# CristianSimion5/vk-raytracing-engine

Hardware: AMD Instinct MI355X
Metric: Mrays/s (higher is better)
Workload: dtype f32

## Files before the change

### include/vkrt.h

```cpp
#ifndef VKRT_H
#define VKRT_H

#include <stdint.h>
#include "vkrt_host_device.h"

#ifdef __cplusplus
extern "C" {
#endif

#define VKRT_ABI_VERSION 4

enum vkrt_status {
  VKRT_OK = 0,
  VKRT_ERR_INVALID_ARGUMENT = 1,
  VKRT_ERR_NO_DEVICE = 2,
  VKRT_ERR_HIP = 3,
  VKRT_ERR_OUT_OF_MEMORY = 4,
  VKRT_ERR_NOT_BUILT = 5,
  VKRT_ERR_UNSUPPORTED = 6
};

typedef struct vkrt_scene vkrt_scene;

typedef struct vkrt_prim_mesh {
// ... 67 lines not shown
typedef struct vkrt_counters {
  uint64_t rays_closest;
  uint64_t rays_shadow;
  uint64_t hits;
  uint64_t diffuse_hits;
  uint64_t tex_taps;
  uint64_t pixels;
  uint64_t nodes_visited;
  uint64_t tris_tested;
  uint64_t wave_node_steps;
  uint64_t wave_tri_steps;
  uint64_t traversal_faults;
  uint64_t pair_records;
} vkrt_counters;

typedef struct vkrt_accel_info {
  uint32_t triangle_count;
  uint32_t node_count;
  uint32_t max_depth;
  uint32_t build_flags;
  float    sah_cost;
  float    build_ms;
  uint64_t node_bytes;
  uint64_t triangle_bytes;
  uint32_t reference_count;
  uint32_t reserved;
} vkrt_accel_info;

int         vkrt_abi_version(void);
const char* vkrt_last_error(void);
int         vkrt_device_count(void);

int  vkrt_scene_create(const vkrt_scene_desc* desc, int device, vkrt_scene** out);
void vkrt_scene_destroy(vkrt_scene* scene);

enum vkrt_option {
  VKRT_OPT_MODE            = 1,
  VKRT_OPT_BVH_LAYOUT      = 2,
  VKRT_OPT_WF_SUBFRAMES    = 3,
  VKRT_OPT_WF_TRAV_BLOCK   = 4,
  VKRT_OPT_WF_SHARE        = 5,
  VKRT_OPT_TRI_THRESHOLD   = 6,
  VKRT_OPT_WF_SHARE_PERIOD = 7,
  VKRT_OPT_WF_SHARE_FLAGS  = 8,
  VKRT_OPT_GBUFFER_MIPS    = 9,
  VKRT_OPT_WATERTIGHT      = 10,
  VKRT_OPT_SKIP_DEAD_SHADOW_RAYS = 11,
  VKRT_OPT_ANYHIT_DISSOLVE = 12,
  VKRT_OPT_WF_FRAMES_IN_FLIGHT = 13,
  VKRT_OPT_SPLIT_BUDGET    = 14,
  VKRT_OPT_LAST            = 14,
  VKRT_OPT_WF_SAMPLE_SYNC  = 15,
  VKRT_OPT_WF_CAMERA_ROUNDS = 16,
  VKRT_INFO_ANYHIT_ORDER   = 100,
  VKRT_INFO_SPLIT_BUDGET   = 101
};
int vkrt_scene_set_option(vkrt_scene* scene, int option, int value);
int vkrt_scene_get_option(const vkrt_scene* scene, int option, int* value);

int vkrt_accel_build(vkrt_scene* scene, uint32_t build_flags, void* hip_stream);
int vkrt_accel_get_info(const vkrt_scene* scene, vkrt_accel_info* out);

int vkrt_scene_update_nodes(vkrt_scene* scene, uint32_t first, uint32_t count, const vkrt_node* nodes, void* hip_stream);
int vkrt_accel_refit(vkrt_scene* scene, void* hip_stream);

enum vkrt_memory { VKRT_MEMORY_HOST = 0, VKRT_MEMORY_DEVICE = 1 };
typedef struct vkrt_vertex_update {
  uint32_t struct_size;
  uint32_t first, count;
  uint32_t memory;
  const float* positions;
  const float* normals;
  const float* tangents;
  const float* texcoords0;
} vkrt_vertex_update;
int vkrt_scene_update_vertices(vkrt_scene* scene, const vkrt_vertex_update* update, void* hip_stream);

typedef struct vkrt_ray {
  float origin[3];    float tmin;
  float direction[3]; float tmax;
} vkrt_ray;
typedef struct vkrt_hit {
  float   t, u, v;
  int32_t instance;
  int32_t primitive;
  int32_t prim_mesh;
  int32_t triangle;
  int32_t material;
} vkrt_hit;
int vkrt_intersect(vkrt_scene* scene, const vkrt_ray* rays, uint32_t n, uint32_t anyhit_seed, vkrt_hit* hits, void* hip_stream);
int vkrt_occluded(vkrt_scene* scene, const vkrt_ray* rays, uint32_t n, uint32_t anyhit_seed, int32_t* occluded, void* hip_stream);

enum vkrt_instance_flags {
  VKRT_INSTANCE_FACING_CULL_DISABLE = 0x1,
  VKRT_INSTANCE_FLIP_FACING = 0x2
};
typedef struct vkrt_instance_visibility {
  uint8_t  mask;
  uint8_t  flags;
  uint16_t reserved;
} vkrt_instance_visibility;
int vkrt_scene_set_instance_visibility(vkrt_scene* scene, uint32_t first, uint32_t count, const vkrt_instance_visibility* vis, void* hip_stream);
int vkrt_scene_get_instance_visibility(const vkrt_scene* scene, uint32_t first, uint32_t count, vkrt_instance_visibility* out);

enum vkrt_ray_flags {
  VKRT_RAY_OPAQUE = 0x1,
// ... 134 lines not shown
```

### vk-raytracing-engine_amd/abi.py

```python
import ctypes as C

c_f = C.c_float
c_i = C.c_int32
c_u = C.c_uint32
c_u64 = C.c_uint64


class Mat4(C.Structure):
    _fields_ = [("m", c_f * 16)]


class GlobalUniforms(C.Structure):
    _fields_ = [("viewProj", Mat4), ("viewInverse", Mat4), ("projInverse", Mat4)]


class PushConstantRay(C.Structure):
    _fields_ = [
        ("clearColor", c_f * 4),
        ("frame", c_i),
        ("lightsCount", c_i),
        ("samples", c_i),
        ("depth", c_i),
        ("useShadows", c_i),
        ("useAO", c_i),
# ... 156 lines not shown
class InstanceVisibility(C.Structure):
    _fields_ = [("mask", C.c_uint8), ("flags", C.c_uint8), ("reserved", C.c_uint16)]


class MaterialAlpha(C.Structure):
    _fields_ = [("mode", c_u), ("cutoff", c_f)]


class QueryOpts(C.Structure):
    _fields_ = [("struct_size", c_u), ("ray_flags", c_u), ("cull_mask", c_u), ("anyhit_seed", c_u)]


class PointQuery(C.Structure):
    _fields_ = [("point", c_f * 3), ("radius", c_f)]


class VertexUpdate(C.Structure):
    _fields_ = [("struct_size", c_u), ("first", c_u), ("count", c_u), ("memory", c_u), ("positions", C.c_void_p), ("normals", C.c_void_p),
                ("tangents", C.c_void_p), ("texcoords0", C.c_void_p)]


assert C.sizeof(VertexUpdate) == 48
assert C.sizeof(Ray) == 32
assert C.sizeof(Hit) == 32
assert C.sizeof(Surface) == 128
assert C.sizeof(InstanceVisibility) == 4
assert C.sizeof(QueryOpts) == 16
assert C.sizeof(MaterialAlpha) == 8

assert C.sizeof(GlobalUniforms) == 192
assert C.sizeof(PushConstantRay) == 44
assert C.sizeof(PrimMeshInfo) == 12
assert C.sizeof(GltfPBRMaterial) == 52
assert C.sizeof(GltfLight) == 32
assert C.sizeof(PrimMesh) == 20
assert C.sizeof(Node) == 68

VKRT_OK, VKRT_ERR_INVALID_ARGUMENT, VKRT_ERR_NO_DEVICE, VKRT_ERR_HIP, VKRT_ERR_OUT_OF_MEMORY, VKRT_ERR_NOT_BUILT, VKRT_ERR_UNSUPPORTED = range(7)
VKRT_BUILD_LBVH_GPU = 0x1
VKRT_BUILD_SAH_HOST = 0x2
VKRT_BUILD_PLOC_GPU = 0x4
VKRT_TRACE_SEED_INDEX_ROW_MAJOR = 0x1
VKRT_TRACE_COUNT_TRAVERSAL = 0x2
VKRT_TRACE_TIME_KERNELS = 0x4
VKRT_TRACE_SAME_SEED_EVERY_FRAME = 0x8
VKRT_ABI_VERSION = 4
VKRT_OPT_MODE, VKRT_OPT_BVH_LAYOUT, VKRT_OPT_WF_SUBFRAMES, VKRT_OPT_WF_TRAV_BLOCK = 1, 2, 3, 4
VKRT_OPT_WF_SHARE, VKRT_OPT_TRI_THRESHOLD, VKRT_OPT_WF_SHARE_PERIOD, VKRT_OPT_WF_SHARE_FLAGS = 5, 6, 7, 8
VKRT_OPT_GBUFFER_MIPS = 9
VKRT_OPT_WATERTIGHT, VKRT_OPT_SKIP_DEAD_SHADOW_RAYS, VKRT_OPT_ANYHIT_DISSOLVE = 10, 11, 12
VKRT_OPT_WF_FRAMES_IN_FLIGHT, VKRT_OPT_SPLIT_BUDGET = 13, 14
VKRT_OPT_WF_SAMPLE_SYNC = 15
VKRT_OPT_WF_CAMERA_ROUNDS = 16
VKRT_INFO_ANYHIT_ORDER = 100
VKRT_INFO_SPLIT_BUDGET = 101
VKRT_INSTANCE_FACING_CULL_DISABLE, VKRT_INSTANCE_FLIP_FACING = 0x1, 0x2
VKRT_RAY_OPAQUE, VKRT_RAY_CULL_BACK_FACING, VKRT_RAY_CULL_FRONT_FACING = 0x1, 0x10, 0x20
VKRT_MEMORY_HOST, VKRT_MEMORY_DEVICE = 0, 1
VKRT_SURFACE_GEOMETRY, VKRT_SURFACE_MATERIAL = 0x1, 0x2
VKRT_ALPHA_OPAQUE, VKRT_ALPHA_MASK = 0, 1
VKRT_MULTIHIT_MAX = 16

VKRT_SYMBOLS = [
    "vkrt_abi_version",
    "vkrt_last_error",
    "vkrt_device_count",
    "vkrt_scene_create",
    "vkrt_scene_destroy",
    "vkrt_scene_set_option",
    "vkrt_scene_get_option",
    "vkrt_reserve",
    "vkrt_reserve_frames",
    "vkrt_accel_build",
    "vkrt_accel_get_info",
    "vkrt_scene_update_nodes",
    "vkrt_accel_refit",
    "vkrt_scene_update_vertices",
    "vkrt_intersect",
    "vkrt_occluded",
    "vkrt_scene_set_instance_visibility",
    "vkrt_scene_get_instance_visibility",
    "vkrt_intersect_ex",
    "vkrt_occluded_ex",
    "vkrt_intersect_multi",
    "vkrt_closest_point",
    "vkrt_hit_surface",
    "vkrt_scene_set_material_alpha",
    "vkrt_scene_get_material_alpha",
    "vkrt_shard_rows",
    "vkrt_pathtrace",
    "vkrt_pathtrace_frames",
    "vkrt_gbuffer_raycast",
    "vkrt_hybrid_trace",
    "vkrt_gbuffer_raycast_nrd",
    "vkrt_hybrid_trace_nrd",
    "vkrt_post",
    "vkrt_denoiser_create",
    "vkrt_denoiser_destroy",
    "vkrt_denoiser_reset",
    "vkrt_denoise_diffuse",
    "vkrt_counters_reset",
    "vkrt_counters_read",
    "vkrt_last_trace_ms",
    "vkrt_last_trace_timing",
    "vkrt_debug_check_accel",
    "vkrt_debug_read_accel",
# ... 109 lines not shown
```

### vk-raytracing-engine_amd/csrc/device_scene.h

```cpp
#pragma once
#include <hip/hip_runtime.h>
#include <stddef.h>
#include <stdint.h>
#include "../../include/vkrt_host_device.h"
#include "device_math.h"

struct DevInstance
{
  float o2w[12];
  float w2o[9];
  int32_t primMesh;
  uint32_t vis;
  int32_t pad;
};
static_assert(sizeof(DevInstance) == 96, "DevInstance");
#define VKRT_VIS_CULL_DISABLE 0x100u
#define VKRT_VIS_FLIP 0x200u
#define VKRT_VIS_MIRRORED 0x10000u

#define VKRT_VERTEX_QUADS 3
#define VKRT_VERTEX_BYTES 48u
struct DevTexRef
{
  uint32_t offset;
  uint32_t wh;
  uint32_t flags;
  uint32_t quads;
};
#define VKRT_TEXREF_BASE 0
#define VKRT_TEXREF_MR 1
#define VKRT_TEXREF_NORMAL 2
#define VKRT_TEXREF_EMISSIVE 3
struct DevMaterial
{
  GltfPBRMaterial m;
  int32_t pad;
  uint32_t alphaMode;
  float alphaCutoff;
  DevTexRef tex[4];
};
static_assert(sizeof(DevMaterial) == 128 && offsetof(DevMaterial, alphaMode) == 56, "DevMaterial");
struct DevShadeMaterial
{
  float f[8];
  uint32_t ref[8];
};
static_assert(sizeof(DevShadeMaterial) == 64, "DevShadeMaterial");

#define VKRT_MAX_MIPS 16
struct DevTexture
{
  uint32_t offset;
  uint32_t width, height;
  uint32_t srgb;
};

#define VKRT_NODE_QUADS 4
#define VKRT_LEAF_MAX 8
#define VKRT_TRAV_DONE ((int)0x80000000)

#define VKRT_TRI_QUADS 3

struct DevScene
{
  const float* positions;
  const uint32_t* indices;
  const float4* vertexPN;
  const DevMaterial* materials;
  const DevShadeMaterial* shadeMaterials;
  const GltfLight* lights;
  const DevInstance* instances;
  const DevTexture* textures;
  const uint32_t* texMips;
  const uint32_t* texels;
  const uint4* texQuads;
  const float* srgbLut;
  const float4* nodes;
  const float4* tris;
  const uint4* triShade;
  uint32_t textureCount;
  uint32_t triCount;
  int32_t rootRef;
  uint32_t stackCap;
  uint32_t layout;
  uint32_t stepLimit;
  uint32_t triThreshold;
  uint32_t sharePeriodMask;
  uint32_t shareMinIdle;
  uint32_t gbufferMips;
  uint32_t shareFlags;
  uint32_t watertight;
  float sceneLo[3], sceneHi[3];
  uint32_t dissolve;
  unsigned long long* faults;
};
struct DevQueryScene : DevScene
{
  const uint2* nodeMasks;
  uint32_t cullMask;
  uint32_t rayFlags;
};
struct DevSurfaceScene : DevScene
{
  const uint4* primMeshes;
  uint32_t instanceCount;
};

#define VKRT_TRAV_FAULT(sc) atomicAdd((sc).faults, 1ull)

#ifndef VKRT_W8_MAX_POSTPONED
#define VKRT_W8_MAX_POSTPONED 8
#endif
// ... 44 lines not shown
```

### vk-raytracing-engine_amd/csrc/traverse_share.h

```cpp
#pragma once
#include "traverse_wide.h"

#define VKRT_SHARE_LDS_WORDS 384
struct ShareRes
{
  unsigned long long* key;
  int* slot;
  float* u;
  float* v;
  int* donor;
};
VKRT_DEV void shareSync()
{
  __builtin_amdgcn_fence(__ATOMIC_RELEASE, "wavefront");
  __builtin_amdgcn_wave_barrier();
  __builtin_amdgcn_fence(__ATOMIC_ACQUIRE, "wavefront");
}
VKRT_DEV ShareRes shareRes(int* lds320)
{
  ShareRes r;
  r.key = (unsigned long long*)lds320; r.slot = lds320 + 128; r.u = (float*)(lds320 + 192); r.v = (float*)(lds320 + 256); r.donor = lds320 + 320;
  return r;
}

template <bool COUNT, bool ANYHIT, int TM = 0>
VKRT_DEV void traverse_wide8_share(const DevScene& sc, bool valid, f3 o, f3 d, float tmin, float tmax, uint2* stk, ShareRes res, RayHit& hit,
                                   TravCount& tc, uint32_t raySeed = 0u)
{
  TriRay<(TM & VKRT_TM_WATERTIGHT) != 0> tr;
  tr.set(d);
  const float4* __restrict__ nodes = sc.nodes;
  const float4* __restrict__ tris = sc.tris;
  const int stride = 64;
  const int cap = (int)(sc.stackCap >> 1);
  const int lane = (int)lane_id();
  const unsigned shareMin = sc.shareMinIdle;
  const unsigned long long below = (1ull << lane) - 1ull;
  bool farFirst = ANYHIT && anyhit_far_first(sc, o, d, tmax);

  res.key[lane] = ((unsigned long long)__float_as_uint(tmax) << 32) | 0xffffffffull;
  res.slot[lane] = -1; res.u[lane] = 0.0f; res.v[lane] = 0.0f;
  shareSync();

  int owner = lane;
  f3 id = mk3(safe_inv(d.x), safe_inv(d.y), safe_inv(d.z));
  bool px = !(id.x < 0.0f), py = !(id.y < 0.0f), pz = !(id.z < 0.0f);
  unsigned oct4 = ((px ? 1u : 0u) | (py ? 2u : 0u) | (pz ? 4u : 0u)) * 0x01010101u;
  uint2 G = make_uint2(0u, (valid && sc.rootRef != VKRT_TRAV_DONE) ? 0x80000000u : 0u);
  uint2 T = make_uint2(0u, 0u);
  int sp = 0, sb = 0, nPost = 0;
  unsigned steps = sc.stepLimit;
  bool busy = G.y != 0u;

  for(unsigned iter = 0;; iter++)
  {
    const unsigned long long busyMask = __ballot(busy);
    if(busyMask == 0ull)
      break;
    if((iter & sc.sharePeriodMask) == sc.sharePeriodMask && (unsigned)__popcll(~busyMask) >= shareMin)
    {
      const bool giveStack = busy && sp - sb >= 1;
      const bool giveChild = (sc.shareFlags & 1u) != 0u && busy && !giveStack && (G.y & 0xff000000u & ((G.y & 0xff000000u) - 1u)) != 0u;
      const bool mayTris = (sc.shareFlags & 16u) != 0u && busy && !giveStack && !giveChild;
      const bool giveParked = mayTris && nPost > 0;
      const bool giveTris = mayTris && !giveParked && (T.y & (T.y - 1u)) != 0u;
      const bool wants = giveStack || giveChild || giveParked || giveTris;
      const unsigned long long donorMask = __ballot(wants), idleMask = ~busyMask;
      if(donorMask != 0ull)
      {
        const unsigned n = min((unsigned)__popcll(donorMask), (unsigned)__popcll(idleMask));
        const unsigned giveRank = (unsigned)__popcll(donorMask & below), takeRank = (unsigned)__popcll(idleMask & below);
        const bool gives = wants && giveRank < n;
        const bool takes = !busy && takeRank < n;
        uint2 e = make_uint2(0u, 0u);
        if(gives)
        {
          if(giveStack)
          {
            e = stk[sb * stride];
            sb++;
          }
          else if(giveChild)
          {
            const unsigned top = G.y & 0xff000000u;
            const unsigned low = farFirst ? (0x80000000u >> (unsigned)__clz((int)top)) : (top & (0u - top));
            e = make_uint2(G.x, low | (G.y & 0xffu));
            G.y &= ~low;
          }
          else if(giveParked)
          {
            e = stk[(cap - nPost) * stride];
            e.x |= 0x80000000u;
            nPost--;
          }
          else
          {
            const unsigned lo = (unsigned)__ffs((int)T.y) - 1u, hi = 31u - (unsigned)__clz((int)T.y);
            const unsigned upper = T.y & ~((1u << ((lo + hi + 1u) >> 1)) - 1u);
            e = make_uint2(T.x | 0x80000000u, upper);
            T.y &= ~upper;
          }
          res.donor[giveRank] = lane;
        }
        shareSync();
        const int src = takes ? res.donor[takeRank] : lane;
        const unsigned ex = (unsigned)__shfl((int)e.x, src), ey = (unsigned)__shfl((int)e.y, src);
        const float ox = __shfl(o.x, src), oy = __shfl(o.y, src), oz = __shfl(o.z, src);
        const float dx = __shfl(d.x, src), dy = __shfl(d.y, src), dz = __shfl(d.z, src);
        const float ix = __shfl(id.x, src), iy = __shfl(id.y, src), iz = __shfl(id.z, src);
        const float tm = __shfl(tmax, src);
        const int ow = __shfl(owner, src);
        if(TM & VKRT_TM_DISSOLVE)
        {
          const uint32_t sd = (uint32_t)__shfl((int)raySeed, src);
          if(takes) raySeed = sd;
        }
        if(takes)
        {
          o = mk3(ox, oy, oz); d = mk3(dx, dy, dz); id = mk3(ix, iy, iz); tmax = tm;
          tr.set(d);
          farFirst = ANYHIT && anyhit_far_first(sc, o, d, tmax);
          px = !(id.x < 0.0f); py = !(id.y < 0.0f); pz = !(id.z < 0.0f);
          oct4 = ((px ? 1u : 0u) | (py ? 2u : 0u) | (pz ? 4u : 0u)) * 0x01010101u;
          if(ex & 0x80000000u)
          {
            G = make_uint2(0u, 0u);
            T = make_uint2(ex & 0x7fffffffu, ey);
          }
          else
          {
            G = make_uint2(ex, ey);
            T = make_uint2(0u, 0u);
          }
          sp = 0; sb = 0; nPost = 0;
          owner = ow;
          steps = sc.stepLimit;
          busy = true;
        }
      }
    }
    shareSync();
    if(busy)
    {
      float bt = tmax;
      int bg = -1;
      bool finished = false;
      bool occluded = false;
      if(ANYHIT)
        finished = __hip_atomic_load(&res.slot[owner], __ATOMIC_RELAXED, __HIP_MEMORY_SCOPE_WAVEFRONT) >= 0;
      else
      {
        const unsigned long long k = __hip_atomic_load(&res.key[owner], __ATOMIC_RELAXED, __HIP_MEMORY_SCOPE_WAVEFRONT);
        bt = __uint_as_float((unsigned)(k >> 32));
        bg = (int)(unsigned)k;
      }
      if(!finished)
      {
        struct Cand
        {
          bool found;
          float t, u, v;
          int slot, gid;
        };
        auto testOne = [&](Cand& cd) {
          const unsigned i = (unsigned)__ffs((int)T.y) - 1u;
          T.y &= T.y - 1u;
          const unsigned s = T.x + i;
          const float4* __restrict__ tp = tris + (size_t)s * VKRT_TRI_QUADS;
          const float4 a = tp[0];
          const float4 b = tp[1];
          const float4 c = tp[2];
          if(COUNT)
          {
            tc.tris++;
            if(lane == __ffsll((long long)__ballot(1)) - 1) tc.waveTriSteps++;
          }
          float t, u, v;
          bool ccw;
          if(tr.hit(o, d, a, b, c, t, u, v, ccw) && t > tmin)
          {
            if(ANYHIT)
            {
              if(t < tmax && !cd.found && !query_rejects<TM>(sc, c, ccw) && !anyhit_ignores<TM>(sc, s, c.y, raySeed, VKRT_HOOK_UV(TM, u, v)))
              {
                cd.found = true; cd.t = t; cd.slot = (int)s;
              }
            }
            else
            {
              const int gid = tri_gid<TM>(c.y);
              const float rt = cd.found ? cd.t : bt;
              const int rg = cd.found ? cd.gid : bg;
              if((t < rt || (t == rt && gid < rg)) && !query_rejects<TM>(sc, c, ccw) && !anyhit_ignores<TM>(sc, s, c.y, raySeed, VKRT_HOOK_UV(TM, u, v)))
              {
                cd.found = true; cd.t = t; cd.u = u; cd.v = v; cd.slot = (int)s; cd.gid = gid;
              }
            }
          }
        };
        auto publish = [&](const Cand& cd) {
          if(!cd.found)
            return;
// ... 30 lines not shown
          {
            if(__builtin_expect(sp + nPost >= cap && nPost > VKRT_W8_POSTPONE_ROOM, 0))
            {
              const uint2 keep = T;
              T = stk[(cap - nPost) * stride];
              nPost--;
              flushT();
              T = keep;
            }
            if(sp + nPost < cap)
            {
              stk[sp * stride] = G;
              sp++;
            }
            else
              VKRT_TRAV_FAULT(sc);
          }
          uint2 Tn;
          w8_test_children<COUNT, (TM & VKRT_TM_FILTER) != 0>(nodes, child, o, id, oct4, px, py, pz, tmin, bt, G, Tn, tc, query_node_masks<TM>(sc),
                                                              query_cull_mask<TM>(sc));
          if(Tn.y != 0u)
          {
            if(T.y != 0u)
            {
              if(__builtin_expect(nPost < VKRT_W8_MAX_POSTPONED && sp + nPost < cap, 1))
              {
                nPost++;
                stk[(cap - nPost) * stride] = T;
              }
              else
              {
                if(!occluded)
                  flushT();
                T.y = 0u;
              }
            }
            T = Tn;
          }
        }
        if((G.y & 0xff000000u) == 0u && sp > sb)
        {
          sp--;
          G = stk[sp * stride];
        }
        if(T.y == 0u && nPost > 0)
        {
          T = stk[(cap - nPost) * stride];
          nPost--;
        }
        bool triStep = true;
        if(sc.triThreshold > 1u)
          triStep = (unsigned)__popcll(__ballot(T.y != 0u)) * 64u >= sc.triThreshold * (unsigned)__popcll(busyMask) ||
                    __ballot((G.y & 0xff000000u) != 0u) == 0ull;
        if(T.y != 0u && triStep && !occluded)
        {
          Cand cd = {false, 0.0f, 0.0f, 0.0f, -1, 0};
          testOne(cd);
          publish(cd);
        }
        if(ANYHIT && occluded)
          finished = true;
        else if((G.y & 0xff000000u) == 0u && T.y == 0u && nPost == 0)
          finished = true;
        else if(--steps == 0u)
        {
          VKRT_TRAV_FAULT(sc);
          finished = true;
        }
      }
      if(finished)
        busy = false;
    }
  }
  shareSync();
  hit.t = __uint_as_float((unsigned)(res.key[lane] >> 32)); hit.u = res.u[lane]; hit.v = res.v[lane]; hit.slot = res.slot[lane];
  if(ANYHIT)
    hit.t = tmax;
}
```

### vk-raytracing-engine_amd/csrc/vkrt_api.cpp

```cpp
#include <hip/hip_runtime.h>

#include <algorithm>
#include <chrono>
#include <cmath>
#include <cstdarg>
#include <cstdio>
#include <cstdlib>
#include <cstring>
#include <initializer_list>
#include <string>
#include <vector>

#include "../../include/vkrt.h"
#include "bvh_host.h"
#include "dev_buffer.h"
#include "device_scene.h"
#include "kernels.h"
#include "wide_node.h"

#define VKRT_TRI_THRESHOLD_DEFAULT 32
#define VKRT_WF_SHARE_DEFAULT 16
#define VKRT_WF_SHARE_FLAGS_DEFAULT 25
#define VKRT_WF_FRAMES_IN_FLIGHT_DEFAULT 3
#define VKRT_SPLIT_BUDGET_DEFAULT -1
#define VKRT_WF_SAMPLE_SYNC_DEFAULT 1
#define VKRT_WF_CAMERA_ROUNDS_DEFAULT 1
#include "lbvh.h"
#include "refit.h"
#include "vertex_update.h"

namespace {

thread_local std::string g_lastError;

int fail(int code, const char* fmt, ...)
{
  char buf[512];
  va_list ap;
  va_start(ap, fmt);
  vsnprintf(buf, sizeof buf, fmt, ap);
  va_end(ap);
  g_lastError = buf;
  return code;
}

#define HIP_TRY(expr)                                                      \
  do                                                                       \
  {                                                                        \
    std::string m_;                                                        \
    if(const int rc_ = vkrt::hip_status((expr), #expr, m_); rc_ != VKRT_OK) \
      return fail(rc_, "%s", m_.c_str());                                  \
  } while(0)

}

struct vkrt_scene
{
  int device = 0;
  int cuCount = 256;
  std::vector<float> positions;
  std::vector<uint32_t> indices;
  std::vector<vkrt_prim_mesh> primMeshes;
  std::vector<vkrt_node> nodes;
  uint32_t lightCount = 0, materialCount = 0;
  std::vector<float> materialAlpha;
  std::vector<void*> allocs;
  DevScene dev{};
  vkrt::TreeBuffers accel;
  bool built = false;
  vkrt_accel_info info{};
  unsigned int* workCounter = nullptr;
  DevCounters* counters = nullptr;
  hipEvent_t evStart = nullptr, evStop = nullptr;
  bool timed = false;
  void* wfMem = nullptr;
  WfBuffers wf{};
  WfAsync wfAsync{};
  std::vector<hipEvent_t> wfEvents;
  WfTiming wfTiming{};
  bool wfTimed = false;
  int splitResolved = 0;
  int wfTimingRounds = 0;
  std::vector<hipEvent_t> wfPool;
  int opt[VKRT_OPT_WF_CAMERA_ROUNDS + 1] = {0, 1, 1, 3, 64, VKRT_WF_SHARE_DEFAULT, VKRT_TRI_THRESHOLD_DEFAULT, 0, VKRT_WF_SHARE_FLAGS_DEFAULT, 1, 0, 0, 0,
                                            VKRT_WF_FRAMES_IN_FLIGHT_DEFAULT, VKRT_SPLIT_BUDGET_DEFAULT, VKRT_WF_SAMPLE_SYNC_DEFAULT, VKRT_WF_CAMERA_ROUNDS_DEFAULT};
  bool hasLargeTriangles = false;
  bool wavefront = true;
  bool stale = false;
  bool refitted = false;
  vkrt::RefitScratch refit;
  bool positionsOnDevice = false;
  vkrt::DevBuf vertexStage;
  size_t vertexStageBytes = 0;
  std::vector<vkrt_instance_visibility> vis;
  uint64_t masksPresent[4] = {0, 0, 0, 0};
  vkrt::DevBuf nodeMasks;
  std::vector<vkrt_material_alpha> alpha;
  uint32_t alphaMasks = 0;
  const uint4* surfacePrimMeshes = nullptr;
};

namespace {

template <typename T>
int upload(vkrt_scene* s, const T* src, size_t count, const T** dst)
{
  void* p = nullptr;
  const size_t bytes = std::max<size_t>(count * sizeof(T), 16);
  HIP_TRY(hipMalloc(&p, bytes));
  s->allocs.push_back(p);
  if(count)
    HIP_TRY(hipMemcpy(p, src, count * sizeof(T), hipMemcpyHostToDevice));
  *dst = (const T*)p;
  return VKRT_OK;
}

int checkTransform(const vkrt_node& n, uint32_t i)
{
  for(int k = 0; k < 16; k++)
    if(!std::isfinite(n.worldMatrix[k]))
      return fail(VKRT_ERR_INVALID_ARGUMENT, "node %u: worldMatrix[%d] is not finite", i, k);
  return VKRT_OK;
}

int validate(const vkrt_scene_desc* d)
{
  if(!d)
    return fail(VKRT_ERR_INVALID_ARGUMENT, "desc is NULL");
  if(d->struct_size != sizeof(vkrt_scene_desc))
    return fail(VKRT_ERR_INVALID_ARGUMENT, "vkrt_scene_desc.struct_size %u != %zu (ABI mismatch)", d->struct_size,
                sizeof(vkrt_scene_desc));
  if(d->vertex_count && (!d->positions || !d->normals || !d->tangents || !d->texcoords0))
    return fail(VKRT_ERR_INVALID_ARGUMENT, "vertex arrays missing");
  if(d->index_count && !d->indices)
    return fail(VKRT_ERR_INVALID_ARGUMENT, "indices missing");
  if(d->material_count == 0 || !d->materials)
    return fail(VKRT_ERR_INVALID_ARGUMENT, "at least one material is required (nvh::GltfScene appends a default one)");
  if(d->light_count == 0 || !d->lights)
// ... 28 lines not shown
    const GltfPBRMaterial& m = d->materials[i];
    const int32_t t[4] = {m.pbrBaseColorTexture, m.metallicRoughnessTexture, m.normalTexture, m.emissiveTexture};
    for(int k = 0; k < 4; k++)
      if(t[k] >= (int32_t)d->texture_count && d->texture_count > 0)
        return fail(VKRT_ERR_INVALID_ARGUMENT, "material %u: texture index %d out of range", i, t[k]);
  }
  for(uint32_t i = 0; i < d->texture_count; i++)
    if(!d->textures[i].rgba8 || d->textures[i].width == 0 || d->textures[i].height == 0)
      return fail(VKRT_ERR_INVALID_ARGUMENT, "texture %u: empty", i);
  return VKRT_OK;
}

float srgbEncode(float c) { return c <= 0.0031308f ? 12.92f * c : 1.055f * powf(c, 1.0f / 2.4f) - 0.055f; }
void downsampleLevel(const uint32_t* src, uint32_t sw, uint32_t sh, uint32_t* dst, uint32_t dw, uint32_t dh, bool srgb, const float* lut512)
{
  for(uint32_t y = 0; y < dh; y++)
    for(uint32_t x = 0; x < dw; x++)
    {
      const float fu = ((float)x + 0.5f) * ((float)sw / (float)dw) - 0.5f, fv = ((float)y + 0.5f) * ((float)sh / (float)dh) - 0.5f;
      const float flx = floorf(fu), fly = floorf(fv), ax = fu - flx, ay = fv - fly;
      auto cl = [](int v, int n) { return v < 0 ? 0 : (v >= n ? n - 1 : v); };
      const int x0 = cl((int)flx, (int)sw), x1 = cl((int)flx + 1, (int)sw), y0 = cl((int)fly, (int)sh), y1 = cl((int)fly + 1, (int)sh);
      const uint32_t p[4] = {src[(size_t)y0 * sw + x0], src[(size_t)y0 * sw + x1], src[(size_t)y1 * sw + x0], src[(size_t)y1 * sw + x1]};
      uint32_t out = 0;
      for(int c = 0; c < 4; c++)
      {
        const uint32_t base = (srgb && c < 3) ? 0u : 256u;
        const float t00 = lut512[base + ((p[0] >> (8 * c)) & 255u)], t10 = lut512[base + ((p[1] >> (8 * c)) & 255u)];
        const float t01 = lut512[base + ((p[2] >> (8 * c)) & 255u)], t11 = lut512[base + ((p[3] >> (8 * c)) & 255u)];
        float v = (t00 * (1.0f - ax) + t10 * ax) * (1.0f - ay) + (t01 * (1.0f - ax) + t11 * ax) * ay;
        if(srgb && c < 3) v = srgbEncode(v);
        v = v < 0.0f ? 0.0f : (v > 1.0f ? 1.0f : v);
        out |= (uint32_t)(v * 255.0f + 0.5f) << (8 * c);
      }
      dst[(size_t)y * dw + x] = out;
    }
}

bool useWavefront(const vkrt_scene* s) { return s->opt[VKRT_OPT_MODE] == 1; }

int clampOption(int option, int v)
{
  switch(option)
  {
    case VKRT_OPT_MODE: case VKRT_OPT_BVH_LAYOUT: return v ? 1 : 0;
    case VKRT_OPT_WF_SUBFRAMES: case VKRT_OPT_WF_FRAMES_IN_FLIGHT: return std::max(1, std::min(VKRT_WF_MAX_LANES, v));
    case VKRT_OPT_SPLIT_BUDGET: return std::max(-1, std::min(100, v));
    case VKRT_OPT_WF_TRAV_BLOCK: return v == 256 ? 256 : v == 128 ? 128 : 64;
    case VKRT_OPT_WF_SHARE: return std::max(0, std::min(64, v));
    case VKRT_OPT_TRI_THRESHOLD: return std::max(0, std::min(65, v));
    case VKRT_OPT_WF_SHARE_PERIOD: return std::max(0, std::min(255, v));
    case VKRT_OPT_WF_SHARE_FLAGS: return v & 31;
    case VKRT_OPT_GBUFFER_MIPS: case VKRT_OPT_WATERTIGHT: case VKRT_OPT_SKIP_DEAD_SHADOW_RAYS: case VKRT_OPT_ANYHIT_DISSOLVE: case VKRT_OPT_WF_SAMPLE_SYNC:
    case VKRT_OPT_WF_CAMERA_ROUNDS: return v ? 1 : 0;
  }
  return v;
}

void optionsFromEnvironment(vkrt_scene* s)
{
  const char* e;
  if((e = getenv("VKRT_MODE")) && !strcmp(e, "mega")) s->opt[VKRT_OPT_MODE] = 0;
  if((e = getenv("VKRT_BVH")) && !strcmp(e, "bvh2")) s->opt[VKRT_OPT_BVH_LAYOUT] = 0;
  const struct { const char* name; int option; } ints[] = {{"VKRT_WF_SUBFRAMES", VKRT_OPT_WF_SUBFRAMES}, {"VKRT_WF_TRAV_BLOCK", VKRT_OPT_WF_TRAV_BLOCK},
                                                          {"VKRT_WF_SHARE", VKRT_OPT_WF_SHARE}, {"VKRT_TRI_THRESHOLD", VKRT_OPT_TRI_THRESHOLD},
                                                          {"VKRT_WF_SHARE_PERIOD", VKRT_OPT_WF_SHARE_PERIOD}, {"VKRT_WF_SHARE_FLAGS", VKRT_OPT_WF_SHARE_FLAGS},
                                                          {"VKRT_GBUFFER_MIPS", VKRT_OPT_GBUFFER_MIPS}, {"VKRT_WATERTIGHT", VKRT_OPT_WATERTIGHT},
                                                          {"VKRT_SKIP_DEAD_SHADOW_RAYS", VKRT_OPT_SKIP_DEAD_SHADOW_RAYS},
                                                          {"VKRT_ANYHIT_DISSOLVE", VKRT_OPT_ANYHIT_DISSOLVE}, {"VKRT_WF_FRAMES_IN_FLIGHT", VKRT_OPT_WF_FRAMES_IN_FLIGHT},
                                                          {"VKRT_SPLIT_BUDGET", VKRT_OPT_SPLIT_BUDGET}, {"VKRT_WF_SAMPLE_SYNC", VKRT_OPT_WF_SAMPLE_SYNC},
                                                          {"VKRT_WF_CAMERA_ROUNDS", VKRT_OPT_WF_CAMERA_ROUNDS}};
  for(const auto& k : ints)
    if((e = getenv(k.name)))
      s->opt[k.option] = clampOption(k.option, atoi(e));
}

void freeAccel(vkrt_scene* s)
{
  s->accel = vkrt::TreeBuffers{};
  s->nodeMasks = vkrt::DevBuf{};
  s->built = false;
  s->refit = vkrt::RefitScratch{};
  s->refitted = false;
  s->stale = false;
}

constexpr vkrt_material_alpha kDefaultAlpha = {VKRT_ALPHA_OPAQUE, 0.5f};
constexpr vkrt_instance_visibility kDefaultVisibility = {0xFF, VKRT_INSTANCE_FACING_CULL_DISABLE, 0};

void makeInstance(const vkrt_node& node, const vkrt_instance_visibility& vis, DevInstance& in)
{
  memset(&in, 0, sizeof in);
  for(int r = 0; r < 3; r++)
    for(int c = 0; c < 4; c++)
      in.o2w[r * 4 + c] = node.worldMatrix[c * 4 + r];
  vkrt::invert3x3_rows(in.o2w, in.w2o);
  in.primMesh = node.primMesh;
  const float* m = in.o2w;
  const double det = (double)m[0] * ((double)m[5] * m[10] - (double)m[6] * m[9]) - (double)m[1] * ((double)m[4] * m[10] - (double)m[6] * m[8]) +
                     (double)m[2] * ((double)m[4] * m[9] - (double)m[5] * m[8]);
  in.vis = (uint32_t)vis.mask | ((uint32_t)vis.flags << 8) | (det < 0.0 ? VKRT_VIS_MIRRORED : 0u);
}

void noteMasks(vkrt_scene* s)
{
  memset(s->masksPresent, 0, sizeof s->masksPresent);
  for(const vkrt_instance_visibility& v : s->vis)
    s->masksPresent[v.mask >> 6] |= 1ull << (v.mask & 63u);
}

bool everyMaskMeets(const vkrt_scene* s, uint32_t cullMask)
{
  for(uint32_t m = 0; m < 256; m++)
    if(((s->masksPresent[m >> 6] >> (m & 63u)) & 1ull) && (m & cullMask) == 0u)
      return false;
  return true;
}

int computeNodeMasks(vkrt_scene* s, hipStream_t stream)
{
  if(s->dev.layout != 1u || !s->nodeMasks.get())
    return VKRT_OK;
  const uint32_t nodes = (uint32_t)(s->info.node_bytes / VKRT_WNODE_BYTES);
  HIP_TRY(vkrt_launch_node_masks(s->dev, nodes, (uint32_t)s->nodes.size(), s->info.max_depth + 1u, s->nodeMasks.get<uint2>(), stream));
// ... 438 lines not shown
  D.stackCap = 1;
  D.layout = 0;
  D.stepLimit = 64;
  D.triThreshold = 0;
  D.shareMinIdle = 0;
  D.sharePeriodMask = 0;
  D.shareFlags = 0;
  D.gbufferMips = 1;

  void* p = nullptr;
  if(hipMalloc(&p, 64) != hipSuccess) return bail(fail(VKRT_ERR_OUT_OF_MEMORY, "hipMalloc(work counter)"));
  s->allocs.push_back(p);
  s->workCounter = (unsigned int*)p;
  if(hipMalloc(&p, sizeof(DevCounters)) != hipSuccess) return bail(fail(VKRT_ERR_OUT_OF_MEMORY, "hipMalloc(counters)"));
  s->allocs.push_back(p);
  s->counters = (DevCounters*)p;
  D.faults = &s->counters->v[0][10];
  if(hipMemset(s->counters, 0, sizeof(DevCounters)) != hipSuccess) return bail(fail(VKRT_ERR_HIP, "hipMemset(counters)"));
  if(hipEventCreate(&s->evStart) != hipSuccess || hipEventCreate(&s->evStop) != hipSuccess)
    return bail(fail(VKRT_ERR_HIP, "hipEventCreate"));
  *out = s;
  return VKRT_OK;
}

void vkrt_scene_destroy(vkrt_scene* s)
{
  if(!s)
    return;
  (void)hipSetDevice(s->device);
  freeAccel(s);
  for(void* p : s->allocs)
    (void)hipFree(p);
  if(s->wfMem) (void)hipFree(s->wfMem);
  if(s->wfAsync.count)
  {
    (void)hipEventDestroy(s->wfAsync.fork);
    for(int j = 0; j < s->wfAsync.count; j++)
    {
      (void)hipStreamDestroy(s->wfAsync.streams[j]);
      (void)hipEventDestroy(s->wfAsync.join[j]);
    }
  }
  for(hipEvent_t e : s->wfEvents) (void)hipEventDestroy(e);
  for(hipEvent_t e : s->wfPool) (void)hipEventDestroy(e);
  if(s->evStart) (void)hipEventDestroy(s->evStart);
  if(s->evStop) (void)hipEventDestroy(s->evStop);
  delete s;
}

int vkrt_scene_set_option(vkrt_scene* s, int option, int value)
{
  if(!s)
    return fail(VKRT_ERR_INVALID_ARGUMENT, "scene is NULL");
  if(option < VKRT_OPT_MODE || option > VKRT_OPT_WF_CAMERA_ROUNDS)
    return fail(VKRT_ERR_INVALID_ARGUMENT, "unknown option %d", option);
  if(clampOption(option, value) != value)
    return fail(VKRT_ERR_INVALID_ARGUMENT, "option %d: value %d out of range", option, value);
  s->opt[option] = value;
  return VKRT_OK;
}

int vkrt_scene_get_option(const vkrt_scene* s, int option, int* value)
{
  if(!s || !value)
    return fail(VKRT_ERR_INVALID_ARGUMENT, "NULL argument");
  if(option == VKRT_INFO_ANYHIT_ORDER)
  {
    *value = s->built ? (int)(s->dev.shareFlags & 6u) : 0;
    return VKRT_OK;
  }
  if(option == VKRT_INFO_SPLIT_BUDGET)
  {
    *value = s->built ? s->splitResolved : 0;
    return VKRT_OK;
  }
  if(option < VKRT_OPT_MODE || option > VKRT_OPT_WF_CAMERA_ROUNDS)
    return fail(VKRT_ERR_INVALID_ARGUMENT, "unknown option %d", option);
  *value = s->opt[option];
  return VKRT_OK;
}

int vkrt_reserve(vkrt_scene* s, const vkrt_shard* shard, void* hip_stream)
{
  if(!s)
    return fail(VKRT_ERR_INVALID_ARGUMENT, "NULL argument");
  return vkrt_reserve_frames(s, shard, (uint32_t)std::max(1, s->opt[VKRT_OPT_WF_FRAMES_IN_FLIGHT]), hip_stream);
}

int vkrt_reserve_frames(vkrt_scene* s, const vkrt_shard* shard, uint32_t frames_per_call, void* hip_stream)
{
  if(!s || !shard)
    return fail(VKRT_ERR_INVALID_ARGUMENT, "NULL argument");
  if(frames_per_call == 0)
    return fail(VKRT_ERR_INVALID_ARGUMENT, "frames_per_call is 0");
  int rc = checkShard(shard);
  if(rc == VKRT_OK)
    rc = setDevice(s);
  if(rc != VKRT_OK)
    return rc;
  const uint64_t tiles = (uint64_t)((shard->full_width + 7) / 8) * ((vkrt_shard_rows(shard) + 7) / 8);
  if(tiles * 64 >= 0xFFFFFFFFull)
    return fail(VKRT_ERR_UNSUPPORTED, "launch too large");
  const bool wavefront = s->built ? s->wavefront : useWavefront(s);
  if(tiles == 0 || !wavefront)
    return VKRT_OK;
  int rc2 = ensureWorkingSet(s, (uint32_t)tiles * 64u, framesInFlight(s, (int)std::min<uint32_t>(frames_per_call, VKRT_FRAMES_PER_BATCH)), (hipStream_t)hip_stream);
  if(rc2 == VKRT_OK)
    rc2 = ensureEventPool(s, (int)std::min<uint32_t>(frames_per_call, VKRT_FRAMES_PER_BATCH));
  return rc2;
}

namespace {

void installTree(vkrt_scene* s, vkrt::BuiltTree& t)
{
  s->accel = std::move(t.buf);
  s->dev.nodes = s->accel.nodes.get<const float4>();
  s->dev.tris = s->accel.tris.get<const float4>();
  s->dev.triShade = s->accel.triShade.get<const uint4>();
  s->dev.layout = t.layout;
  s->dev.rootRef = t.rootRef;
  s->dev.stackCap = t.layout == 1 ? 2 * (t.maxDepth + 1) : t.maxDepth + 2;
  s->info.node_count = t.nodeCount;
  s->info.max_depth = t.maxDepth;
  s->info.sah_cost = t.sahCost;
  s->info.node_bytes = t.nodeBytes;
  s->info.triangle_bytes = t.triangleBytes;
}

// ... 50 lines not shown
      {
        const float w = n.worldMatrix[k] * p[0] + n.worldMatrix[4 + k] * p[1] + n.worldMatrix[8 + k] * p[2] + n.worldMatrix[12 + k];
        lo[k] = std::min(lo[k], w); hi[k] = std::max(hi[k], w);
      }
    }
  }
  for(int k = 0; k < 3; k++)
  {
    const float pad = 1e-3f * std::max(1e-6f, hi[k] - lo[k]);
    s->dev.sceneLo[k] = lo[k] - pad; s->dev.sceneHi[k] = hi[k] + pad;
  }
  const double ex = (double)hi[0] - lo[0], ey = (double)hi[1] - lo[1], ez = (double)hi[2] - lo[2];
  const double face = std::max(ex * ey, std::max(ey * ez, ez * ex));
  double maxArea = 0.0;
  for(const vkrt_node& n : s->nodes)
  {
    const vkrt_prim_mesh& pm = s->primMeshes[(size_t)n.primMesh];
    const float* M = n.worldMatrix;
    for(uint32_t t = 0; t + 3 <= pm.indexCount; t += 3)
    {
      double w[3][3];
      for(int v = 0; v < 3; v++)
      {
        const float* p = &s->positions[3 * (size_t)(s->indices[pm.firstIndex + t + v] + pm.vertexOffset)];
        for(int k = 0; k < 3; k++) w[v][k] = (double)M[k] * p[0] + (double)M[4 + k] * p[1] + (double)M[8 + k] * p[2] + (double)M[12 + k];
      }
      const double a[3] = {w[1][0] - w[0][0], w[1][1] - w[0][1], w[1][2] - w[0][2]}, b[3] = {w[2][0] - w[0][0], w[2][1] - w[0][1], w[2][2] - w[0][2]};
      const double cx = a[1] * b[2] - a[2] * b[1], cy = a[2] * b[0] - a[0] * b[2], cz = a[0] * b[1] - a[1] * b[0];
      maxArea = std::max(maxArea, 0.5 * std::sqrt(cx * cx + cy * cy + cz * cz));
    }
  }
  s->hasLargeTriangles = face > 0.0 && maxArea > 0.01 * face;
}

int traversalSettings(vkrt_scene* s)
{
  s->info.reference_count = s->dev.triCount;
  s->dev.stepLimit = 4u * (s->info.node_count + s->dev.triCount) + 64u;
  s->dev.triThreshold = 0;
  s->dev.shareMinIdle = 0;
  s->dev.sharePeriodMask = 0;
  s->dev.shareFlags = (uint32_t)s->opt[VKRT_OPT_WF_SHARE_FLAGS] & 6u;
  const bool largeWhole = s->hasLargeTriangles && s->info.reference_count == s->info.triangle_count;
  if((s->opt[VKRT_OPT_WF_SHARE_FLAGS] & 8) && !largeWhole)
    s->dev.shareFlags |= 4u;
  if(s->dev.layout == 1)
  {
    s->dev.triThreshold = (uint32_t)s->opt[VKRT_OPT_TRI_THRESHOLD];
    if(s->dev.triThreshold != 0u)
      s->dev.stackCap += 2 * VKRT_W8_POSTPONE_ROOM;
    s->dev.shareMinIdle = (uint32_t)s->opt[VKRT_OPT_WF_SHARE];
    s->dev.sharePeriodMask = (uint32_t)s->opt[VKRT_OPT_WF_SHARE_PERIOD];
    s->dev.shareFlags |= (uint32_t)s->opt[VKRT_OPT_WF_SHARE_FLAGS] & 17u;
  }
  if((size_t)s->dev.stackCap * 256 * 4 > 64 * 1024)
    return fail(VKRT_ERR_UNSUPPORTED, "BVH depth %u needs a %zu-byte LDS stack per workgroup (limit 64 KiB)", s->info.max_depth,
                (size_t)s->dev.stackCap * 256 * 4);
  return VKRT_OK;
}

int accelBuildOnce(vkrt_scene* s, uint32_t flags, int splitBudget, hipStream_t stream)
{
  if(flags == 0)
    flags = VKRT_BUILD_DEFAULT;
  const bool wantPloc = (flags & VKRT_BUILD_PLOC_GPU) != 0;
  const bool wantLbvh = (flags & VKRT_BUILD_LBVH_GPU) != 0 || wantPloc, wantSah = (flags & VKRT_BUILD_SAH_HOST) != 0;
  if(wantLbvh == wantSah || (wantPloc && (flags & VKRT_BUILD_LBVH_GPU) != 0) || (flags & ~7u) != 0)
    return fail(VKRT_ERR_INVALID_ARGUMENT, "build_flags must select exactly one of VKRT_BUILD_LBVH_GPU / VKRT_BUILD_PLOC_GPU / VKRT_BUILD_SAH_HOST");
  int rc = setDevice(s);
  if(rc != VKRT_OK)
    return rc;
  HIP_TRY(hipStreamSynchronize(stream));
  freeAccel(s);
  const auto t0 = std::chrono::steady_clock::now();
  s->info = vkrt_accel_info{};
  s->info.build_flags = wantPloc ? VKRT_BUILD_PLOC_GPU : wantLbvh ? VKRT_BUILD_LBVH_GPU : VKRT_BUILD_SAH_HOST;
  s->wavefront = useWavefront(s);
  const bool watertight = s->opt[VKRT_OPT_WATERTIGHT] != 0;
  if((watertight || s->opt[VKRT_OPT_ANYHIT_DISSOLVE] != 0) && useWavefront(s) && s->opt[VKRT_OPT_WF_TRAV_BLOCK] != 64)
    return fail(VKRT_ERR_UNSUPPORTED, "VKRT_OPT_WATERTIGHT / VKRT_OPT_ANYHIT_DISSOLVE are built for the default 64-thread traversal workgroups "
                "(VKRT_OPT_WF_TRAV_BLOCK = %d)", s->opt[VKRT_OPT_WF_TRAV_BLOCK]);
  std::vector<uint8_t> instDissolves;
  bool dissolve = false;
  if(s->opt[VKRT_OPT_ANYHIT_DISSOLVE] != 0)
    for(const vkrt_node& n : s->nodes)
    {
      const int32_t m = std::max(0, s->primMeshes[(size_t)n.primMesh].materialIndex);
      const bool nonOpaque = s->materialAlpha[(size_t)m] < 1.0f && s->primMeshes[(size_t)n.primMesh].indexCount >= 3u;
      instDissolves.push_back(nonOpaque ? 1 : 0);
      dissolve = dissolve || nonOpaque;
    }
  s->dev.watertight = watertight ? 1u : 0u;
  s->dev.dissolve = dissolve ? 1u : 0u;
  const std::vector<uint8_t>* dissolvePtr = dissolve ? &instDissolves : nullptr;
  const bool wide = useWavefront(s) && s->opt[VKRT_OPT_BVH_LAYOUT] == 1;

  vkrt::BuiltTree tree;
  if(wantSah)
  {
    std::vector<vkrt::FlatTri> tris;
    vkrt::flatten_instances(s->positions.data(), s->indices.data(), s->primMeshes.data(), s->nodes.data(),
                            (uint32_t)s->nodes.size(), tris);
    vkrt::BuiltBvh bvh;
    vkrt::BuiltWide8 w8;
    if(wide)
      vkrt::build_wide8_host(tris, w8, watertight);
// ... 1165 lines not shown
```

Before: 5392.

## Lend pending leaf triangles from busy lanes to idle lanes during traversal

Adds a triangle-lending step to the wave-shared traversal. On a triangle step, lanes holding several pending leaf triangles give their highest one to an idle lane, which tests it against the lender's ray (fetched by shuffle) and writes the hit result into the shared per-ray key or slot. Idle lanes stay in the loop when lending is on. The feature is enabled by default through a new option and shareFlags bit. It aims to cut SIMD divergence during leaf testing, at the cost of extra ballots, shuffles, LDS atomics and barriers on every triangle step.

```diff
diff --git a/include/vkrt.h b/include/vkrt.h
--- a/include/vkrt.h
+++ b/include/vkrt.h
@@ -143,6 +143,7 @@
   VKRT_OPT_LAST            = 14,
   VKRT_OPT_WF_SAMPLE_SYNC  = 15,
   VKRT_OPT_WF_CAMERA_ROUNDS = 16,
+  VKRT_OPT_WF_TRI_LEND = 17,
   VKRT_INFO_ANYHIT_ORDER   = 100,
   VKRT_INFO_SPLIT_BUDGET   = 101
 };
diff --git a/vk-raytracing-engine_amd/abi.py b/vk-raytracing-engine_amd/abi.py
--- a/vk-raytracing-engine_amd/abi.py
+++ b/vk-raytracing-engine_amd/abi.py
@@ -232,6 +232,7 @@
 VKRT_OPT_WF_FRAMES_IN_FLIGHT, VKRT_OPT_SPLIT_BUDGET = 13, 14
 VKRT_OPT_WF_SAMPLE_SYNC = 15
 VKRT_OPT_WF_CAMERA_ROUNDS = 16
+VKRT_OPT_WF_TRI_LEND = 17
 VKRT_INFO_ANYHIT_ORDER = 100
 VKRT_INFO_SPLIT_BUDGET = 101
 VKRT_INSTANCE_FACING_CULL_DISABLE, VKRT_INSTANCE_FLIP_FACING = 0x1, 0x2
diff --git a/vk-raytracing-engine_amd/csrc/device_scene.h b/vk-raytracing-engine_amd/csrc/device_scene.h
--- a/vk-raytracing-engine_amd/csrc/device_scene.h
+++ b/vk-raytracing-engine_amd/csrc/device_scene.h
@@ -58,6 +58,7 @@
 #define VKRT_NODE_QUADS 4
 #define VKRT_LEAF_MAX 8
 #define VKRT_TRAV_DONE ((int)0x80000000)
+#define VKRT_SHARE_TRI_LEND 0x20u
 
 #define VKRT_TRI_QUADS 3
 
diff --git a/vk-raytracing-engine_amd/csrc/traverse_share.h b/vk-raytracing-engine_amd/csrc/traverse_share.h
--- a/vk-raytracing-engine_amd/csrc/traverse_share.h
+++ b/vk-raytracing-engine_amd/csrc/traverse_share.h
@@ -15,6 +15,10 @@
   __builtin_amdgcn_fence(__ATOMIC_RELEASE, "wavefront");
   __builtin_amdgcn_wave_barrier();
   __builtin_amdgcn_fence(__ATOMIC_ACQUIRE, "wavefront");
+}
+VKRT_DEV unsigned laneRank(unsigned long long mask)
+{
+  return __builtin_amdgcn_mbcnt_hi((unsigned)(mask >> 32), __builtin_amdgcn_mbcnt_lo((unsigned)mask, 0u));
 }
 VKRT_DEV ShareRes shareRes(int* lds320)
 {
@@ -35,7 +39,6 @@
   const int cap = (int)(sc.stackCap >> 1);
   const int lane = (int)lane_id();
   const unsigned shareMin = sc.shareMinIdle;
-  const unsigned long long below = (1ull << lane) - 1ull;
   bool farFirst = ANYHIT && anyhit_far_first(sc, o, d, tmax);
 
   res.key[lane] = ((unsigned long long)__float_as_uint(tmax) << 32) | 0xffffffffull;
@@ -51,6 +54,7 @@
   int sp = 0, sb = 0, nPost = 0;
   unsigned steps = sc.stepLimit;
   bool busy = G.y != 0u;
+  const bool lendOn = (TM & (VKRT_TM_WATERTIGHT | VKRT_TM_DISSOLVE)) != (VKRT_TM_WATERTIGHT | VKRT_TM_DISSOLVE) && (sc.shareFlags & VKRT_SHARE_TRI_LEND) != 0u;
 
   for(unsigned iter = 0;; iter++)
   {
@@ -69,7 +73,7 @@
       if(donorMask != 0ull)
       {
         const unsigned n = min((unsigned)__popcll(donorMask), (unsigned)__popcll(idleMask));
-        const unsigned giveRank = (unsigned)__popcll(donorMask & below), takeRank = (unsigned)__popcll(idleMask & below);
+        const unsigned giveRank = laneRank(donorMask), takeRank = laneRank(idleMask);
         const bool gives = wants && giveRank < n;
         const bool takes = !busy && takeRank < n;
         uint2 e = make_uint2(0u, 0u);
@@ -140,14 +144,14 @@
       }
     }
     shareSync();
-    if(busy)
+    if(busy || lendOn)
     {
       float bt = tmax;
       int bg = -1;
       bool finished = false;
       bool occluded = false;
       if(ANYHIT)
-        finished = __hip_atomic_load(&res.slot[owner], __ATOMIC_RELAXED, __HIP_MEMORY_SCOPE_WAVEFRONT) >= 0;
+        finished = busy && __hip_atomic_load(&res.slot[owner], __ATOMIC_RELAXED, __HIP_MEMORY_SCOPE_WAVEFRONT) >= 0;
       else
       {
         const unsigned long long k = __hip_atomic_load(&res.key[owner], __ATOMIC_RELAXED, __HIP_MEMORY_SCOPE_WAVEFRONT);
@@ -284,7 +288,93 @@
         if(sc.triThreshold > 1u)
           triStep = (unsigned)__popcll(__ballot(T.y != 0u)) * 64u >= sc.triThreshold * (unsigned)__popcll(busyMask) ||
                     __ballot((G.y & 0xff000000u) != 0u) == 0ull;
-        if(T.y != 0u && triStep && !occluded)
+        bool lentStep = false;
+        if(lendOn && triStep)
+        {
+          const bool tests = T.y != 0u && !occluded;
+          const unsigned rest1 = T.y & (T.y - 1u);
+          const bool multi = rest1 != 0u && !occluded, isFree = T.y == 0u && !occluded;
+          const unsigned long long lendMask = __ballot(multi), freeMask = __ballot(isFree);
+          const unsigned n = min((unsigned)__popcll(lendMask), (unsigned)__popcll(freeMask));
+          if(n != 0u)
+          {
+            lentStep = true;
+            const unsigned lendRank = laneRank(lendMask), freeRank = laneRank(freeMask);
+            const bool borrows = isFree && freeRank < n;
+            unsigned s = 0u, ls = 0u;
+            if(multi && lendRank < n)
+            {
+              const unsigned hi = 31u - (unsigned)__clz((int)T.y);
+              T.y &= ~(1u << hi);
+              ls = T.x + hi;
+              res.donor[lendRank] = lane;
+            }
+            if(tests)
+            {
+              s = T.x + (unsigned)__ffs((int)T.y) - 1u;
+              T.y &= T.y - 1u;
+            }
+            shareSync();
+            const int src = borrows ? res.donor[freeRank] : lane;
+            const unsigned bs = (unsigned)__shfl((int)ls, src);
+            const f3 ro = mk3(__shfl(o.x, src), __shfl(o.y, src), __shfl(o.z, src));
+            const f3 rd = mk3(__shfl(d.x, src), __shfl(d.y, src), __shfl(d.z, src));
+            const int row = __shfl(owner, src);
+            const float rbt = __shfl(bt, src);
+            const int rbg = ANYHIT ? 0 : __shfl(bg, src);
+            uint32_t rseed = raySeed;
+            if(TM & VKRT_TM_DISSOLVE)
+              rseed = (uint32_t)__shfl((int)raySeed, src);
+            if(tests || borrows)
+            {
+              if(borrows)
+              {
+                s = bs;
+                tr.set(rd);
+              }
+              const float4* __restrict__ tp = tris + (size_t)s * VKRT_TRI_QUADS;
+              const float4 a = tp[0];
+              const float4 b = tp[1];
+              const float4 c = tp[2];
+              if(COUNT)
+              {
+                tc.tris++;
+                if(lane == __ffsll((long long)__ballot(1)) - 1) tc.waveTriSteps++;
+              }
+              float t, u, v;
+              bool ccw;
+              if(tr.hit(ro, rd, a, b, c, t, u, v, ccw) && t > tmin)
+              {
+                if(ANYHIT)
+                {
+                  if(t < rbt && !query_rejects<TM>(sc, c, ccw) && !anyhit_ignores<TM>(sc, s, c.y, rseed, VKRT_HOOK_UV(TM, u, v)))
+                  {
+                    __hip_atomic_store(&res.slot[row], (int)s, __ATOMIC_RELAXED, __HIP_MEMORY_SCOPE_WAVEFRONT);
+                    if(!borrows)
+                      occluded = true;
+                  }
+                }
+                else
+                {
+                  const int gid = tri_gid<TM>(c.y);
+                  if((t < rbt || (t == rbt && gid < rbg)) && !query_rejects<TM>(sc, c, ccw) && !anyhit_ignores<TM>(sc, s, c.y, rseed, VKRT_HOOK_UV(TM, u, v)))
+                  {
+                    const unsigned long long mine = ((unsigned long long)__float_as_uint(t) << 32) | (unsigned)gid;
+                    __hip_atomic_fetch_min(&res.key[row], mine, __ATOMIC_RELAXED, __HIP_MEMORY_SCOPE_WAVEFRONT);
+                    shareSync();
+                    if(__hip_atomic_load(&res.key[row], __ATOMIC_RELAXED, __HIP_MEMORY_SCOPE_WAVEFRONT) == mine)
+                    {
+                      res.slot[row] = (int)s; res.u[row] = u; res.v[row] = v;
+                    }
+                  }
+                }
+              }
+              if((TM & VKRT_TM_WATERTIGHT) != 0 && borrows)
+                tr.set(d);
+            }
+          }
+        }
+        if(!lentStep && T.y != 0u && triStep && !occluded)
         {
           Cand cd = {false, 0.0f, 0.0f, 0.0f, -1, 0};
           testOne(cd);
@@ -301,7 +391,13 @@
         }
       }
       if(finished)
+      {
+        if(lendOn && busy)
+        {
+          G.y = 0u; T.y = 0u; sp = 0; sb = 0; nPost = 0;
+        }
         busy = false;
+      }
     }
   }
   shareSync();
diff --git a/vk-raytracing-engine_amd/csrc/vkrt_api.cpp b/vk-raytracing-engine_amd/csrc/vkrt_api.cpp
--- a/vk-raytracing-engine_amd/csrc/vkrt_api.cpp
+++ b/vk-raytracing-engine_amd/csrc/vkrt_api.cpp
@@ -25,6 +25,7 @@
 #define VKRT_SPLIT_BUDGET_DEFAULT -1
 #define VKRT_WF_SAMPLE_SYNC_DEFAULT 1
 #define VKRT_WF_CAMERA_ROUNDS_DEFAULT 1
+#define VKRT_WF_TRI_LEND_DEFAULT 1
 #include "lbvh.h"
 #include "refit.h"
 #include "vertex_update.h"
@@ -82,8 +83,9 @@
   int splitResolved = 0;
   int wfTimingRounds = 0;
   std::vector<hipEvent_t> wfPool;
-  int opt[VKRT_OPT_WF_CAMERA_ROUNDS + 1] = {0, 1, 1, 3, 64, VKRT_WF_SHARE_DEFAULT, VKRT_TRI_THRESHOLD_DEFAULT, 0, VKRT_WF_SHARE_FLAGS_DEFAULT, 1, 0, 0, 0,
-                                            VKRT_WF_FRAMES_IN_FLIGHT_DEFAULT, VKRT_SPLIT_BUDGET_DEFAULT, VKRT_WF_SAMPLE_SYNC_DEFAULT, VKRT_WF_CAMERA_ROUNDS_DEFAULT};
+  int opt[VKRT_OPT_WF_TRI_LEND + 1] = {0, 1, 1, 3, 64, VKRT_WF_SHARE_DEFAULT, VKRT_TRI_THRESHOLD_DEFAULT, 0, VKRT_WF_SHARE_FLAGS_DEFAULT, 1, 0, 0, 0,
+                                            VKRT_WF_FRAMES_IN_FLIGHT_DEFAULT, VKRT_SPLIT_BUDGET_DEFAULT, VKRT_WF_SAMPLE_SYNC_DEFAULT, VKRT_WF_CAMERA_ROUNDS_DEFAULT,
+                                      VKRT_WF_TRI_LEND_DEFAULT};
   bool hasLargeTriangles = false;
   bool wavefront = true;
   bool stale = false;
@@ -218,7 +220,7 @@
     case VKRT_OPT_WF_SHARE_PERIOD: return std::max(0, std::min(255, v));
     case VKRT_OPT_WF_SHARE_FLAGS: return v & 31;
     case VKRT_OPT_GBUFFER_MIPS: case VKRT_OPT_WATERTIGHT: case VKRT_OPT_SKIP_DEAD_SHADOW_RAYS: case VKRT_OPT_ANYHIT_DISSOLVE: case VKRT_OPT_WF_SAMPLE_SYNC:
-    case VKRT_OPT_WF_CAMERA_ROUNDS: return v ? 1 : 0;
+    case VKRT_OPT_WF_CAMERA_ROUNDS: case VKRT_OPT_WF_TRI_LEND: return v ? 1 : 0;
   }
   return v;
 }
@@ -235,7 +237,8 @@
                                                           {"VKRT_SKIP_DEAD_SHADOW_RAYS", VKRT_OPT_SKIP_DEAD_SHADOW_RAYS},
                                                           {"VKRT_ANYHIT_DISSOLVE", VKRT_OPT_ANYHIT_DISSOLVE}, {"VKRT_WF_FRAMES_IN_FLIGHT", VKRT_OPT_WF_FRAMES_IN_FLIGHT},
                                                           {"VKRT_SPLIT_BUDGET", VKRT_OPT_SPLIT_BUDGET}, {"VKRT_WF_SAMPLE_SYNC", VKRT_OPT_WF_SAMPLE_SYNC},
-                                                          {"VKRT_WF_CAMERA_ROUNDS", VKRT_OPT_WF_CAMERA_ROUNDS}};
+                                                          {"VKRT_WF_CAMERA_ROUNDS", VKRT_OPT_WF_CAMERA_ROUNDS},
+                                                          {"VKRT_WF_TRI_LEND", VKRT_OPT_WF_TRI_LEND}};
   for(const auto& k : ints)
     if((e = getenv(k.name)))
       s->opt[k.option] = clampOption(k.option, atoi(e));
@@ -780,11 +783,13 @@
 {
   if(!s)
     return fail(VKRT_ERR_INVALID_ARGUMENT, "scene is NULL");
-  if(option < VKRT_OPT_MODE || option > VKRT_OPT_WF_CAMERA_ROUNDS)
+  if(option < VKRT_OPT_MODE || option > VKRT_OPT_WF_TRI_LEND)
     return fail(VKRT_ERR_INVALID_ARGUMENT, "unknown option %d", option);
   if(clampOption(option, value) != value)
     return fail(VKRT_ERR_INVALID_ARGUMENT, "option %d: value %d out of range", option, value);
   s->opt[option] = value;
+  if(option == VKRT_OPT_WF_TRI_LEND && s->built && s->dev.layout == 1u)
+    s->dev.shareFlags = (s->dev.shareFlags & ~VKRT_SHARE_TRI_LEND) | (value ? VKRT_SHARE_TRI_LEND : 0u);
   return VKRT_OK;
 }
 
@@ -802,7 +807,7 @@
     *value = s->built ? s->splitResolved : 0;
     return VKRT_OK;
   }
-  if(option < VKRT_OPT_MODE || option > VKRT_OPT_WF_CAMERA_ROUNDS)
+  if(option < VKRT_OPT_MODE || option > VKRT_OPT_WF_TRI_LEND)
     return fail(VKRT_ERR_INVALID_ARGUMENT, "unknown option %d", option);
   *value = s->opt[option];
   return VKRT_OK;
@@ -959,6 +964,8 @@
     s->dev.shareMinIdle = (uint32_t)s->opt[VKRT_OPT_WF_SHARE];
     s->dev.sharePeriodMask = (uint32_t)s->opt[VKRT_OPT_WF_SHARE_PERIOD];
     s->dev.shareFlags |= (uint32_t)s->opt[VKRT_OPT_WF_SHARE_FLAGS] & 17u;
+    if(s->opt[VKRT_OPT_WF_TRI_LEND])
+      s->dev.shareFlags |= VKRT_SHARE_TRI_LEND;
   }
   if((size_t)s->dev.stackCap * 256 * 4 > 64 * 1024)
     return fail(VKRT_ERR_UNSUPPORTED, "BVH depth %u needs a %zu-byte LDS stack per workgroup (limit 64 KiB)", s->info.max_depth,
```

After: 5449, median of 6. 1.1% higher.
